# nunofachada/cl_ops

Measured on AMD Instinct MI355X. Metric: Mkeys/s sorting 2^28 uint32 (satradix, 4-bit digits); achieved % of HBM roofline, higher is better.
Workload: dtype u32

## Files before the change

cl_ops_amd/csrc/hip/clo_hip_radix1.hip:

```cpp
#include <hip/hip_runtime.h>

#include <cstdio>
#include <cstdlib>

#include "clo_hip.h"
#include "clo_hip_internal.h"
#include "clo_hip_radix_rank.h"

namespace {

constexpr int R1_PEEL = 4;
constexpr int R1_WINDOW = 8;
constexpr unsigned R1_VALID = 0x80000000u;
constexpr int R1_CNT_SHIFT = 40;
constexpr clo_u64 R1_SUM_MASK = (1ull << R1_CNT_SHIFT) - 1ull;
constexpr int R1_ROW = 256;
constexpr int R1_POOLS = 8;
constexpr int R1_TICKET_STRIDE = 16;
constexpr int R1_GH_THREADS = 512;

__device__ __forceinline__ unsigned r1_ld32(const unsigned* p) {
	return __hip_atomic_load(p, __ATOMIC_RELAXED, __HIP_MEMORY_SCOPE_AGENT);
}
__device__ __forceinline__ void r1_st32(unsigned* p, unsigned v) {
	__hip_atomic_store(p, v, __ATOMIC_RELAXED, __HIP_MEMORY_SCOPE_AGENT);
}

template <typename E, int NP>
__global__ __launch_bounds__(R1_GH_THREADS)
void clo_radix1_ghist_kernel(const E* __restrict__ in, size_t n, unsigned key_shift, unsigned key_bits,
	unsigned* __restrict__ ghist, unsigned* __restrict__ gbase, unsigned* __restrict__ done,
	int aligned, clo_keyx kx, unsigned tiles_per_group) {
	constexpr int ITEMS = sweep_shape<E>::ITEMS;
	constexpr int TILE = R1_GH_THREADS * ITEMS;
	constexpr int COPIES = NP <= 4 ? 32 : 16;
	__shared__ unsigned s_cnt[NP * (R1_ROW / 2) * COPIES];
	const unsigned tid = threadIdx.x, cp = tid & (COPIES - 1);
	for (unsigned i = tid; i < (unsigned) (NP * (R1_ROW / 2) * COPIES); i += R1_GH_THREADS) s_cnt[i] = 0;
	__syncthreads();
	const unsigned last_bits = key_bits - 8u * (NP - 1);
	const unsigned last_mask = (1u << last_bits) - 1u;
	const size_t tile0 = (size_t) blockIdx.x * tiles_per_group;
	for (unsigned t = 0; t < tiles_per_group; ++t) {
		const size_t base = (tile0 + t) * TILE;
		if (base >= n) break;
		const unsigned count = (n - base) < (size_t) TILE ? (unsigned) (n - base) : (unsigned) TILE;
		const unsigned tbase = tid * ITEMS;
		E key[ITEMS];
		if (count == (unsigned) TILE) {
			load_blocked<E, ITEMS>(in + base + tbase, key, aligned != 0);
		} else {
			#pragma unroll
			for (int i = 0; i < ITEMS; ++i) key[i] = (tbase + i < count) ? in[base + tbase + i] : (E) 0;
		}
		#pragma unroll
		for (int i = 0; i < ITEMS; ++i) {
			if (count == (unsigned) TILE || tbase + i < count) {
				const E k = clo_keyx_fwd<E>(key[i], kx) >> key_shift;
				#pragma unroll
				for (int p = 0; p < NP; ++p) {
					const unsigned d = (unsigned) (k >> (8 * p)) & (p == NP - 1 ? last_mask : 255u);
					atomicAdd(&s_cnt[((unsigned) p * (R1_ROW / 2) + (d >> 1)) * COPIES + cp], 1u << ((d & 1u) * 16u));
				}
			}
		}
	}
	__syncthreads();
	for (unsigned i = tid; i < (unsigned) (NP * R1_ROW / 2); i += R1_GH_THREADS) {
		unsigned even = 0, odd = 0;
		#pragma unroll
		for (int c = 0; c < COPIES; ++c) {
			const unsigned x = s_cnt[i * COPIES + ((c + i) & (COPIES - 1))];
			even += x & 0xffffu;
			odd += x >> 16;
		}
		if (even) atomicAdd(&ghist[2 * i], even);
		if (odd) atomicAdd(&ghist[2 * i + 1], odd);
	}
	__shared__ unsigned s_last, s_w[4];
	asm volatile("s_waitcnt vmcnt(0)" ::: "memory");
	__syncthreads();
	if (tid == 0) s_last = atomicAdd(done, 1u) == gridDim.x - 1u;
	__syncthreads();
	if (!s_last) return;
	const unsigned lane = tid & 63u, wave = tid >> 6;
	for (int p = 0; p < NP; ++p) {
		unsigned v = 0, incl = 0;
		if (tid < (unsigned) R1_ROW) {
			v = __hip_atomic_load(&ghist[p * R1_ROW + tid], __ATOMIC_RELAXED, __HIP_MEMORY_SCOPE_AGENT);
			incl = clo_wave_scan_inclusive<unsigned>(v, lane);
			if (lane == 63) s_w[wave] = incl;
		}
		__syncthreads();
		if (tid < (unsigned) R1_ROW) {
			unsigned b = incl - v;
			#pragma unroll
			for (unsigned w = 0; w < 4; ++w) if (w < wave) b += s_w[w];
			gbase[p * R1_ROW + tid] = b;
		}
		__syncthreads();
	}
}

struct r1_pass {
	unsigned* agg;
	clo_u64* cacc;
	unsigned* cprefix;
	unsigned* ticket;
	const unsigned* gbase;
	unsigned* status;
	clo_u64* stamps;
	unsigned tiles, max_spins;
	unsigned pools;
};

template <typename E, int LB, int HB, int R1_CHUNK_LOG, int R1_EARLY>
__global__ __launch_bounds__(sweep_shape<E>::THREADS, 6)
void clo_radix1_sweep_kernel(const E* __restrict__ in, E* __restrict__ out, size_t n,
	unsigned shift, unsigned mask_lo, unsigned mask_hi, r1_pass P, int aligned, clo_keyx kx_in, clo_keyx kx_out) {

	constexpr int THREADS = sweep_shape<E>::THREADS;
	constexpr int ITEMS = sweep_shape<E>::ITEMS;
	constexpr int TILE = THREADS * ITEMS;
	constexpr int WAVES = THREADS / 64;
	constexpr int R2 = 1 << (LB + HB);
	constexpr int HMAX = pc_words<(LB > HB ? LB : HB)>::H;
	constexpr unsigned R1_CHUNK = 1u << R1_CHUNK_LOG;
	static_assert(R1_EARLY <= (int) R1_CHUNK, "at most the whole level 1");
	static_assert(R2 <= R1_ROW && R2 <= THREADS, "one thread per combined digit");
	static_assert(THREADS >= 2 * R1_ROW, "the digit threads are the second half of the work-group");

	__shared__ __attribute__((aligned(16))) E s_stage[TILE];
	__shared__ unsigned s_end[THREADS * PC_END_STRIDE];
	__shared__ unsigned s_wtot[WAVES][HMAX];
	__shared__ __attribute__((aligned(16))) unsigned s_wbase[WAVES][HMAX];
	__shared__ unsigned s_delta[R2];
	__shared__ unsigned s_w4[4];
	__shared__ unsigned s_tile;

	const unsigned tid = threadIdx.x, lane = tid & 63u, wave = tid >> 6;
	clo_u64 t0 = 0, t1 = 0, t2 = 0, t3 = 0, t4 = 0, t5 = 0;
	if (P.stamps) t0 = __builtin_amdgcn_s_memtime();

	const int dg = (int) tid - (THREADS - R1_ROW);
	const bool dthread = dg >= 0 && dg < R2;
	const bool dwaves = wave >= (unsigned) (WAVES - R1_ROW / 64);
	const unsigned dwave = wave - (unsigned) (WAVES - R1_ROW / 64);

	unsigned* s_hist = reinterpret_cast<unsigned*>(s_stage);
	static_assert(sizeof(E) * TILE >= WAVES * R1_ROW * sizeof(unsigned), "the histogram fits the stage");
	#pragma unroll
	for (int k = 0; k < WAVES * R1_ROW / THREADS; ++k) s_hist[k * THREADS + tid] = 0;

	if (tid == 0) {
		const unsigned nchunks = (P.tiles + R1_CHUNK - 1u) >> R1_CHUNK_LOG;
		const unsigned x = clo_xcc_id();
		unsigned tile = 0xffffffffu;
		for (unsigned t = 0; t < P.pools; ++t) {
			const unsigned pool = (x + t) & (P.pools - 1u);
			const unsigned k = atomicAdd(&P.ticket[pool * R1_TICKET_STRIDE], 1u);
			const unsigned c = (k >> R1_CHUNK_LOG) * P.pools + pool;
			const unsigned cand = (c << R1_CHUNK_LOG) + (k & (R1_CHUNK - 1u));
			if (c < nchunks && cand < P.tiles) { tile = cand; break; }
		}
		s_tile = tile;
	}
	clo_lds_barrier();
	const unsigned tile = s_tile;
	if (tile == 0xffffffffu) return;
	const unsigned c = tile >> R1_CHUNK_LOG, q = tile & (R1_CHUNK - 1u);
	const unsigned in_chunk = P.tiles - (c << R1_CHUNK_LOG) < R1_CHUNK ? P.tiles - (c << R1_CHUNK_LOG) : R1_CHUNK;
	const size_t base = (size_t) tile * TILE;
	const unsigned count = (n - base) < (size_t) TILE ? (unsigned) (n - base) : (unsigned) TILE;
	const bool full = count == (unsigned) TILE;
	const unsigned tbase = tid * ITEMS;
	const unsigned mask2 = (mask_hi << LB) | mask_lo;
	const unsigned n32 = (unsigned) n;

	E key[ITEMS];
	if (full) {
		load_blocked<E, ITEMS>(in + base + tbase, key, aligned != 0);
	} else {
		#pragma unroll
		for (int i = 0; i < ITEMS; ++i) key[i] = (tbase + i < count) ? in[base + tbase + i] : (E) 0;
	}
	if (kx_in.kind) {
		#pragma unroll
		for (int i = 0; i < ITEMS; ++i) key[i] = clo_keyx_fwd<E>(key[i], kx_in);
	}
	if (P.stamps) t1 = __builtin_amdgcn_s_memtime();
	{
		const unsigned d0 = (unsigned) (key[0] >> shift) & mask2;
		const bool skewed = __popcll(__ballot(d0 == (unsigned) __builtin_amdgcn_readfirstlane((int) d0))) >= 16;
		unsigned* const row = s_hist + wave * R1_ROW;
		if (!skewed) {
			#pragma unroll
			for (int i = 0; i < ITEMS; ++i)
				if (full || tbase + i < count) atomicAdd(&row[(unsigned) (key[i] >> shift) & mask2], 1u);
		} else {
			#pragma unroll
			for (int i = 0; i < ITEMS; ++i) {
				const unsigned d = (unsigned) (key[i] >> shift) & mask2;
				bool mine = full || tbase + i < count;
				#pragma unroll 1
				for (int r = 0; r < R1_PEEL; ++r) {
					const unsigned long long rem = __ballot(mine);
					if (rem == 0) break;
					const int l = __ffsll((long long) rem) - 1;
					const unsigned dl = (unsigned) __builtin_amdgcn_readlane((int) d, l);
					const bool grp = mine && d == dl;
					const unsigned cnt = (unsigned) __popcll(__ballot(grp));
					if ((int) lane == l) atomicAdd(&row[dl], cnt);
					mine = mine && !grp;
				}
				if (mine) atomicAdd(&row[d], 1u);
			}
		}
	}

	unsigned h2 = 0, incl2 = 0;
	clo_u64 old = 0;
	auto publish = [&]() {
		if (!dwaves) return;
		if (dthread) {
			#pragma unroll
			for (int w = 0; w < WAVES; ++w) h2 += s_hist[w * R1_ROW + dg];
			r1_st32(&P.agg[(size_t) tile * R1_ROW + dg], R1_VALID | h2);
			old = __hip_atomic_fetch_add(&P.cacc[(size_t) c * R1_ROW + dg], (1ull << R1_CNT_SHIFT) | (clo_u64) h2,
				__ATOMIC_RELAXED, __HIP_MEMORY_SCOPE_AGENT);
		}
		incl2 = clo_wave_scan_inclusive<unsigned>(h2, lane);
		if (lane == 63) s_w4[dwave] = incl2;
	};
	pc_local_split<E, LB, THREADS, ITEMS, HMAX>(key, shift, mask_lo, count, s_stage, s_end, s_wtot, s_wbase, publish);
	if (P.stamps) t2 = __builtin_amdgcn_s_memtime();

	unsigned dstart2 = 0;
	unsigned early[R1_EARLY > 0 ? R1_EARLY : 1];
	#pragma unroll
	for (unsigned k = 0; k < (unsigned) R1_EARLY; ++k) early[k] = (k == 0 ? c > 0 : k <= q) ? 0u : R1_VALID;
	if (dthread) {
		dstart2 = incl2 - h2;
		#pragma unroll
		for (unsigned w = 0; w < 4; ++w) if (w < dwave) dstart2 += s_w4[w];
		if ((unsigned) (old >> R1_CNT_SHIFT) == in_chunk - 1u) {
			const clo_u64 total = (old & R1_SUM_MASK) + h2;
			clo_u64 excl = 0;
			long j = (long) c - 1;
			unsigned spins = 0;
			while (j >= 0) {
				unsigned pv[R1_WINDOW];
				clo_u64 av[R1_WINDOW];
				#pragma unroll
				for (int w = 0; w < R1_WINDOW; ++w) {
					pv[w] = 0; av[w] = 0;
					if (j - w >= 0) {
						pv[w] = r1_ld32(&P.cprefix[(size_t) (j - w) * R1_ROW + dg]);
						av[w] = clo_ld_agent(&P.cacc[(size_t) (j - w) * R1_ROW + dg]);
					}
				}
				bool closed = false, stalled = false;
				int used = 0;
				#pragma unroll
				for (int w = 0; w < R1_WINDOW; ++w) {
					if (closed || stalled || j - w < 0) continue;
					if (pv[w] & R1_VALID) { excl += pv[w] & ~R1_VALID; closed = true; }
					else if ((unsigned) (av[w] >> R1_CNT_SHIFT) == R1_CHUNK) { excl += av[w] & R1_SUM_MASK; used = w + 1; }
					else stalled = true;
				}
				if (closed) break;
				j -= used;
				if (stalled) {
					if (++spins > P.max_spins) { atomicExch(P.status, 1u); break; }
					__builtin_amdgcn_s_sleep(2);
				}
			}
			r1_st32(&P.cprefix[(size_t) c * R1_ROW + dg], R1_VALID | (unsigned) (excl + total));
		}
	}
	if (P.stamps) t3 = __builtin_amdgcn_s_memtime();

	if (mask_hi != 0) {
		if (full) {
			constexpr int PER = ITEMS * (int) sizeof(E) >= 16 ? 16 / (int) sizeof(E) : ITEMS;
			typedef E vec16 __attribute__((ext_vector_type(PER)));
			#pragma unroll
			for (int k = 0; k < ITEMS / PER; ++k) {
				const vec16 t = *reinterpret_cast<const vec16*>(&s_stage[tbase + k * PER]);
				#pragma unroll
				for (int qq = 0; qq < PER; ++qq) key[k * PER + qq] = t[qq];
			}
		} else {
			#pragma unroll
			for (int i = 0; i < ITEMS; ++i) if (tbase + i < count) key[i] = s_stage[tbase + i];
		}
		auto request = [&]() {
			if (!dthread) return;
			#pragma unroll
			for (unsigned k = 0; k < (unsigned) R1_EARLY; ++k) {
				const bool want = k == 0 ? c > 0 : k <= q;
				const unsigned* a = !want ? &P.agg[(size_t) tile * R1_ROW + dg]
					: (k == 0 ? &P.cprefix[(size_t) (c - 1) * R1_ROW + dg] : &P.agg[(size_t) (tile - k) * R1_ROW + dg]);
				early[k] = r1_ld32(a);
			}
		};
		pc_local_split<E, HB, THREADS, ITEMS, HMAX>(key, shift + LB, mask_hi, count, s_stage, s_end, s_wtot, s_wbase, request);
	}
	if (P.stamps) t4 = __builtin_amdgcn_s_memtime();

	if (dthread) {
		const unsigned* addr[R1_CHUNK];
		unsigned v[R1_CHUNK];
		#pragma unroll
		for (unsigned k = 0; k < R1_CHUNK; ++k) {
			const bool want = k == 0 ? c > 0 : k <= q;
			addr[k] = !want ? &P.agg[(size_t) tile * R1_ROW + dg]
				: (k == 0 ? &P.cprefix[(size_t) (c - 1) * R1_ROW + dg] : &P.agg[(size_t) (tile - k) * R1_ROW + dg]);
			v[k] = k < (unsigned) R1_EARLY ? early[k] : (want ? 0u : R1_VALID);
		}
		unsigned spins = 0;
		for (;;) {
			bool all = true;
			#pragma unroll
			for (unsigned k = 0; k < R1_CHUNK; ++k) all = all && (v[k] & R1_VALID);
			if (all) break;
			if (spins != 0) __builtin_amdgcn_s_sleep(1);
			if (++spins > P.max_spins) { atomicExch(P.status, 1u); break; }
			#pragma unroll
			for (unsigned g = 0; g < R1_CHUNK / 4; ++g) {
				if (g != 0 && q < 4 * g) continue;
				if (spins == 1 && 4 * g + 3 < (unsigned) R1_EARLY) {
					const bool have = (v[4 * g] & v[4 * g + 1] & v[4 * g + 2] & v[4 * g + 3] & R1_VALID) != 0;
					if (__builtin_amdgcn_ballot_w64(!have) == 0) continue;
				}
				unsigned nv[4];
				#pragma unroll
				for (unsigned k = 0; k < 4; ++k) nv[k] = r1_ld32(addr[4 * g + k]);
				#pragma unroll
				for (unsigned k = 0; k < 4; ++k) if (!(v[4 * g + k] & R1_VALID)) v[4 * g + k] = nv[k];
			}
		}
		#pragma unroll
		for (unsigned k = 0; k < R1_CHUNK; ++k) {
			const bool want = k == 0 ? c > 0 : k <= q;
			if (!want) v[k] = R1_VALID;
		}
		unsigned excl = 0;
		#pragma unroll
		for (unsigned k = 0; k < R1_CHUNK; ++k) excl += v[k] & ~R1_VALID;
		s_delta[dg] = P.gbase[dg] + excl - dstart2;
	}
	clo_lds_barrier();
	if (P.stamps) t5 = __builtin_amdgcn_s_memtime();

	constexpr int VEC = sizeof(E) >= 8 ? 1 : 4;
	typedef E vecE __attribute__((ext_vector_type(VEC)));
	typedef E vecE_u __attribute__((ext_vector_type(VEC), aligned(sizeof(E))));
	#pragma unroll
	for (int j = 0; j < ITEMS / VEC; ++j) {
		const unsigned p = (j * THREADS + tid) * VEC;
		if (full) {
			const vecE vv = *reinterpret_cast<const vecE*>(&s_stage[p]);
			const unsigned d0 = (unsigned) (vv[0] >> shift) & mask2, dl = (unsigned) (vv[VEC - 1] >> shift) & mask2;
			const unsigned gi0 = p + s_delta[d0];
			if (d0 == dl && gi0 <= n32 - VEC) {
				vecE vo = vv;
				if (kx_out.kind) {
					#pragma unroll
					for (int k = 0; k < VEC; ++k) vo[k] = clo_keyx_inv<E>(vv[k], kx_out);
				}
				*reinterpret_cast<vecE_u*>(&out[gi0]) = vo;
			} else {
				#pragma unroll
				for (int k = 0; k < VEC; ++k) {
					const unsigned gi = p + k + s_delta[(unsigned) (vv[k] >> shift) & mask2];
					if (gi < n32) out[gi] = clo_keyx_inv<E>(vv[k], kx_out);
				}
			}
		} else {
			#pragma unroll
			for (int k = 0; k < VEC; ++k) {
				if (p + k < count) {
					const E e = s_stage[p + k];
					const unsigned gi = p + k + s_delta[(unsigned) (e >> shift) & mask2];
					if (gi < n32) out[gi] = clo_keyx_inv<E>(e, kx_out);
				}
			}
		}
	}
	if (P.stamps && tid == 0) {
		clo_u64* st = P.stamps + (size_t) tile * 8;
		st[0] = t0; st[1] = t1; st[2] = t2; st[3] = t3; st[4] = t4; st[5] = t5;
		st[6] = __builtin_amdgcn_s_memtime();
		st[7] = ((clo_u64) clo_xcc_id() << 32) | blockIdx.x;
	}
}

struct r1_layout { size_t ghist, gbase, tickets, done, pass0, per_pass, agg, cacc, cprefix, total, tiles, chunks; int passes; };

r1_layout r1_make_layout(size_t n, int elem_size, int key_bits) {
	r1_layout L;
	const size_t tile = (size_t) 512 * (elem_size == 8 ? 8 : 16);
	L.tiles = (n + tile - 1) / tile;
	if (L.tiles == 0) L.tiles = 1;
	L.chunks = (L.tiles + 7) / 8;
	L.passes = (key_bits + 7) / 8;
	size_t off = 0;
	L.ghist = off; off += (size_t) L.passes * R1_ROW * sizeof(unsigned);
	L.gbase = off; off += (size_t) L.passes * R1_ROW * sizeof(unsigned);
	L.tickets = off; off += (size_t) L.passes * R1_POOLS * R1_TICKET_STRIDE * sizeof(unsigned);
	L.done = off; off += 64;
	off = (off + 255) & ~(size_t) 255;
	L.pass0 = off;
	L.agg = 0;
	L.cacc = L.agg + L.tiles * R1_ROW * sizeof(unsigned);
	L.cprefix = L.cacc + L.chunks * R1_ROW * sizeof(clo_u64);
	L.per_pass = (L.cprefix + L.chunks * R1_ROW * sizeof(unsigned) + 255) & ~(size_t) 255;
	L.total = L.pass0 + L.per_pass * (size_t) L.passes;
	return L;
}

int r1_device_cus() {
	int dev = 0, cus = 0;
	if (hipGetDevice(&dev) != hipSuccess) return 0;
	if (hipDeviceGetAttribute(&cus, hipDeviceAttributeMultiprocessorCount, dev) != hipSuccess) return 0;
	return cus;
}

clo_u64* g_r1_stamps = nullptr;
size_t g_r1_stamps_tiles = 0;

template <typename E, int NP>
void r1_launch_ghist(const E* src, size_t n, int key_shift, int key_bits, unsigned* ghist, unsigned* gbase, unsigned* done,
	clo_keyx kx, unsigned tiles, hipStream_t s) {
	unsigned per = tiles > 4096u ? (tiles + 2047u) / 2048u : (tiles > 256u ? 2u : 1u);
	if (per > 16u) per = 16u;
	const unsigned groups = (tiles + per - 1u) / per;
	hipLaunchKernelGGL((clo_radix1_ghist_kernel<E, NP>), dim3(groups), dim3(R1_GH_THREADS), 0, s,
		src, n, (unsigned) key_shift, (unsigned) key_bits, ghist, gbase, done, (int) ((uintptr_t) src % 16 == 0), kx, per);
}

template <typename E>
int r1_sort_impl(const E* src, E* dst, E* tmp, size_t n, int key_shift, int key_bits, clo_keyx kx, void* ws, unsigned* status, hipStream_t s) {
	const r1_layout L = r1_make_layout(n, (int) sizeof(E), key_bits);
	char* w = (char*) ws;
	unsigned* ghist = (unsigned*) (w + L.ghist);
	unsigned* gbase = (unsigned*) (w + L.gbase);
	unsigned* tickets = (unsigned*) (w + L.tickets);
	const unsigned tiles = (unsigned) L.tiles;
	const int passes = L.passes;
	const clo_keyx kx_none = { 0, 0, 0 };
	const clo_hip_env_t* env = clo_hip_env();
	const unsigned max_spins = env->max_spins;

	unsigned pools = (tiles > 1024u && r1_device_cus() >= 256) ? (unsigned) R1_POOLS : 1u;
	if (env->r1_pools != 0) pools = env->r1_pools == R1_POOLS ? (unsigned) R1_POOLS : 1u;

	hipError_t e = hipMemsetAsync(ws, 0, L.total, s);
	if (e != hipSuccess) return (int) e;
	{
		clo_timing_scope timing("radix_ghist", s);
		switch (passes) {
			#define CLO_R1_GH(NP) case NP: r1_launch_ghist<E, NP>(src, n, key_shift, key_bits, ghist, gbase, (unsigned*) (w + L.done), kx, tiles, s); break
			CLO_R1_GH(1); CLO_R1_GH(2); CLO_R1_GH(3); CLO_R1_GH(4); CLO_R1_GH(5); CLO_R1_GH(6); CLO_R1_GH(7); CLO_R1_GH(8);
			#undef CLO_R1_GH
			default: return CLO_HIP_EUNSUPPORTED;
		}
	}
	const bool inplace_odd = (dst == src) && (passes % 2 == 1);
	const E* cur_in = src;
	for (int p = 0; p < passes; ++p) {
		E* cur_out;
		if (inplace_odd) cur_out = (p % 2 == 0) ? tmp : dst;
		else cur_out = ((passes - 1 - p) % 2 == 0) ? dst : tmp;
		const int rem = key_bits - p * 8;
		const int bits = rem < 8 ? rem : 8;
		const int lo_bits = bits < 4 ? bits : 4, hi_bits = bits - lo_bits;
		char* pw = w + L.pass0 + (size_t) p * L.per_pass;
		r1_pass P;
		P.agg = (unsigned*) (pw + L.agg);
		P.cacc = (clo_u64*) (pw + L.cacc);
		P.cprefix = (unsigned*) (pw + L.cprefix);
		P.ticket = tickets + (size_t) p * R1_POOLS * R1_TICKET_STRIDE;
		P.gbase = gbase + (size_t) p * R1_ROW;
		P.status = status;
		P.stamps = (g_r1_stamps && g_r1_stamps_tiles >= L.tiles && p == passes - 1) ? g_r1_stamps : nullptr;
		P.tiles = tiles;
		P.max_spins = max_spins;
		P.pools = pools;
		clo_timing_scope timing("radix_sweep", s);
		#define CLO_R1_SWEEP(CL, EARLY) hipLaunchKernelGGL((clo_radix1_sweep_kernel<E, 4, 4, CL, EARLY>), dim3(tiles), dim3(sweep_shape<E>::THREADS), 0, s, \
			cur_in, cur_out, n, (unsigned) (key_shift + p * 8), (1u << lo_bits) - 1u, (1u << hi_bits) - 1u, P, \
			(int) ((uintptr_t) cur_in % 16 == 0), p == 0 ? kx : kx_none, p + 1 == passes ? kx : kx_none)
		CLO_R1_SWEEP(4, 8);
		#undef CLO_R1_SWEEP
		cur_in = cur_out;
	}
	e = hipGetLastError();
	if (e != hipSuccess) return (int) e;
	if (inplace_odd) {
		e = hipMemcpyAsync(dst, tmp, n * sizeof(E), hipMemcpyDeviceToDevice, s);
		if (e != hipSuccess) return (int) e;
	}
	return 0;
}

}

int clo_radix1_applies(size_t n, int elem_size, int digit_bits) {
	const int mode = clo_hip_env()->radix_sweep;
	if (mode == 0) return 0;
	if ((digit_bits != 4 && digit_bits != 8) || (elem_size != 4 && elem_size != 8) || n >= 0x80000000ull) return 0;
	const size_t tiles = (n + (size_t) 512 * (elem_size == 8 ? 8 : 16) - 1) / ((size_t) 512 * (elem_size == 8 ? 8 : 16));
	if (mode == 1) return tiles > 1;
	return tiles >= 2 && tiles <= 256;
}

size_t clo_radix1_workspace_bytes(size_t n, int elem_size, int key_bits) {
	return r1_make_layout(n, elem_size, key_bits).total;
}

int clo_radix1_sort(const void* src, void* dst, void* tmp, size_t n, int elem_size, int key_shift, int key_bits,
	clo_keyx kx, void* ws, unsigned* status, hipStream_t s) {
	if (elem_size == 4) return r1_sort_impl<uint32_t>((const uint32_t*) src, (uint32_t*) dst, (uint32_t*) tmp, n, key_shift, key_bits, kx, ws, status, s);
	if (elem_size == 8) return r1_sort_impl<uint64_t>((const uint64_t*) src, (uint64_t*) dst, (uint64_t*) tmp, n, key_shift, key_bits, kx, ws, status, s);
	return CLO_HIP_EUNSUPPORTED;
}

extern "C" int clo_hip_radix_debug_stamps(void* buffer, size_t tiles) {
	g_r1_stamps = (clo_u64*) buffer;
	g_r1_stamps_tiles = buffer ? tiles : 0;
	return 0;
}
```

cl_ops_amd/csrc/hip/clo_hip_radix4.hip:

```cpp
#include <hip/hip_runtime.h>

#include <cstdlib>
#include <type_traits>

#include "clo_hip.h"
#include "clo_hip_internal.h"
#include "clo_hip_radix_rank.h"

namespace {

template <int KB> struct kv_key;
template <> struct kv_key<1> { typedef uint8_t type; };
template <> struct kv_key<2> { typedef uint16_t type; };
template <> struct kv_key<4> { typedef uint32_t type; };

template <int KB, int ITEMS>
__device__ __forceinline__ void kv_load_pairs(const clo_kv_io& kv, size_t at, unsigned valid, bool aligned, uint64_t (&pair)[ITEMS]) {
	typedef typename kv_key<KB>::type K;
	const K* kp = reinterpret_cast<const K*>(kv.keys_in) + at;
	K k[ITEMS];
	unsigned v[ITEMS];
	if (valid == (unsigned) ITEMS) {
		load_blocked<K, ITEMS>(kp, k, aligned);
		if (kv.values_in) {
			load_blocked<unsigned, ITEMS>(kv.values_in + at, v, aligned);
		} else {
			#pragma unroll
			for (int i = 0; i < ITEMS; ++i) v[i] = (unsigned) at + (unsigned) i;
		}
	} else {
		#pragma unroll
		for (int i = 0; i < ITEMS; ++i) {
			k[i] = (unsigned) i < valid ? kp[i] : (K) 0;
			v[i] = (unsigned) i < valid ? (kv.values_in ? kv.values_in[at + i] : (unsigned) at + (unsigned) i) : 0u;
		}
	}
	#pragma unroll
	for (int i = 0; i < ITEMS; ++i) pair[i] = ((uint64_t) k[i] << 32) | v[i];
}

template <int KB>
__device__ __forceinline__ void kv_store_pair(const clo_kv_io& kv, unsigned gi, uint64_t e) {
	typedef typename kv_key<KB>::type K;
	if (kv.keys_out) reinterpret_cast<K*>(kv.keys_out)[gi] = (K) (e >> 32);
	kv.values_out[gi] = (unsigned) e;
}

template <typename E, int LB, int HB, bool BIG, bool DIG = false, bool SEG = false, int KV_IN = 0, int KV_OUT = 0>
__global__ __launch_bounds__((pair_shape<E, BIG>::THREADS), (pair_shape<E, BIG>::THREADS >= 1024 ? 8 : 6))
void clo_radix4_pair_kernel(const E* __restrict__ in, E* __restrict__ out, size_t n,
	unsigned shift, unsigned mask_lo, unsigned mask_hi,
	const unsigned* __restrict__ thist, const unsigned* __restrict__ toff, const unsigned* __restrict__ dbase,
	const unsigned* __restrict__ tinfo, int aligned,
	clo_keyx kx_in, clo_keyx kx_out, unsigned char* __restrict__ dig_out = nullptr, unsigned next_shift = 0,
	const clo_seg_tile* __restrict__ tdesc = nullptr, const E* __restrict__ in2 = nullptr, clo_kv_io kv = clo_kv_io()) {
	static_assert((KV_IN == 0 && KV_OUT == 0) || (sizeof(E) == 8 && !SEG), "key-value passes: 8-byte pairs, one array");

	constexpr int THREADS = pair_shape<E, BIG>::THREADS;
	constexpr int ITEMS = pair_shape<E, BIG>::ITEMS;
	constexpr int TILE = THREADS * ITEMS;
	constexpr int WAVES = THREADS / 64;
	constexpr int R2 = 1 << (LB + HB);
	constexpr int HMAX = pc_words<(LB > HB ? LB : HB)>::H;
	static_assert(R2 <= 256 && R2 <= THREADS, "one thread per combined digit, scanned by the first four waves");

	__shared__ __attribute__((aligned(16))) E s_stage[TILE];
	constexpr bool ALIAS = pair_shape<E, BIG>::ALIAS;
	__shared__ unsigned s_end[ALIAS ? 1 : THREADS * PC_END_STRIDE];
	__shared__ unsigned s_wtot[WAVES][HMAX];
	__shared__ __attribute__((aligned(16))) unsigned s_wbase[WAVES][HMAX];
	__shared__ unsigned s_delta[R2];
	__shared__ unsigned s_w4[4];

	const unsigned tid = threadIdx.x, lane = tid & 63u, wave = tid >> 6;
	const unsigned per_xcd = SEG ? (unsigned) ((n + 7) / 8) : (unsigned) ((n + (size_t) TILE * 8 - 1) / ((size_t) TILE * 8));
	const unsigned tile = (blockIdx.x & 7u) * per_xcd + (blockIdx.x >> 3);
	size_t base = (size_t) tile * TILE;
	unsigned count, n32;
	if constexpr (SEG) {
		if (tile >= (unsigned) n) return;
		const clo_seg_tile td = tdesc[tile];
		base = (size_t) td.in_base;
		count = td.count_seg & 0xffffu;
		n32 = td.seg_n;
		out += td.out_base;
		if constexpr (DIG) dig_out += td.out_base;
		dbase += (size_t) ((td.count_seg >> 16) & 0x7fffu) * R2;
		if (td.count_seg >> 31) in = in2;
	} else {
		if (base >= n) return;
		count = (n - base) < (size_t) TILE ? (unsigned) (n - base) : (unsigned) TILE;
		n32 = n > 0xffffffffull ? 0xffffffffu : (unsigned) n;
	}
	const bool full = count == (unsigned) TILE;
	const unsigned tbase = tid * ITEMS;
	const unsigned mask2 = (mask_hi << LB) | mask_lo;

	__builtin_amdgcn_s_setprio(3);
	unsigned h2 = 0, goff = 0;
	if (tid < (unsigned) R2) {
		h2 = thist[(size_t) tile * R2 + tid];
		goff = toff[(size_t) tile * R2 + tid];
		if (dbase) goff += dbase[tid];
	}
	E key[ITEMS];
	if constexpr (KV_IN != 0) {
		kv_load_pairs<KV_IN, ITEMS>(kv, base + tbase, full ? (unsigned) ITEMS : (count > tbase ? count - tbase : 0u), aligned != 0, key);
	} else if (full) {
		if constexpr (SEG) load_blocked_unaligned<E, ITEMS>(in + base + tbase, key);
		else load_blocked<E, ITEMS>(in + base + tbase, key, aligned != 0);
	} else {
		#pragma unroll
		for (int i = 0; i < ITEMS; ++i) key[i] = (tbase + i < count) ? in[base + tbase + i] : (E) 0;
	}
	__builtin_amdgcn_s_setprio(0);
	if (kx_in.kind) {
		#pragma unroll
		for (int i = 0; i < ITEMS; ++i) key[i] = clo_keyx_fwd<E>(key[i], kx_in);
	}
	{
		const unsigned incl2 = clo_wave_scan_inclusive<unsigned>(h2, lane);
		if (lane == 63 && wave < 4) s_w4[wave] = incl2;
		if (tid < (unsigned) R2) s_delta[tid] = goff - (incl2 - h2);
	}

	const bool single = tinfo[tile] != 0u;

	if (!single) {
		pc_local_split<E, LB, THREADS, ITEMS, HMAX, pc_no_mid, pc_no_counted, ALIAS>(key, shift, mask_lo, count, s_stage, s_end, s_wtot, s_wbase);
	} else {
		if (full) {
			constexpr int PER = ITEMS * (int) sizeof(E) >= 16 ? 16 / (int) sizeof(E) : ITEMS;
			typedef E vec16 __attribute__((ext_vector_type(PER)));
			#pragma unroll
			for (int k = 0; k < ITEMS / PER; ++k) {
				vec16 t;
				#pragma unroll
				for (int q = 0; q < PER; ++q) t[q] = key[k * PER + q];
				*reinterpret_cast<vec16*>(&s_stage[tbase + k * PER]) = t;
			}
		} else {
			#pragma unroll
			for (int i = 0; i < ITEMS; ++i) if (tbase + i < count) s_stage[tbase + i] = key[i];
		}
		clo_lds_barrier();
	}

	if (tid < (unsigned) R2) {
		unsigned before = 0;
		#pragma unroll
		for (unsigned w = 0; w < 4; ++w) if (w < wave) before += s_w4[w];
		s_delta[tid] -= before;
	}
	if (single) {
		__syncthreads();
	} else if (mask_hi != 0) {
		if (full) {
			constexpr int PER = ITEMS * (int) sizeof(E) >= 16 ? 16 / (int) sizeof(E) : ITEMS;
			typedef E vec16 __attribute__((ext_vector_type(PER)));
			#pragma unroll
			for (int k = 0; k < ITEMS / PER; ++k) {
				const vec16 t = *reinterpret_cast<const vec16*>(&s_stage[tbase + k * PER]);
				#pragma unroll
				for (int q = 0; q < PER; ++q) key[k * PER + q] = t[q];
			}
		} else {
			#pragma unroll
			for (int i = 0; i < ITEMS; ++i) if (tbase + i < count) key[i] = s_stage[tbase + i];
		}
		pc_local_split<E, HB, THREADS, ITEMS, HMAX, pc_no_mid, pc_no_counted, ALIAS>(key, shift + LB, mask_hi, count, s_stage, s_end, s_wtot, s_wbase);
	} else {
		__syncthreads();
	}

	constexpr int VEC = sizeof(E) >= 8 ? 1 : 4;
	typedef E vecE __attribute__((ext_vector_type(VEC)));
	typedef E vecE_u __attribute__((ext_vector_type(VEC), aligned(sizeof(E))));
	const bool dig_bytes = DIG && VEC == 4 && (next_shift & 7u) == 0u && next_shift < 8u * (unsigned) sizeof(E);
	const unsigned dig_b = next_shift >> 3;
	const unsigned dig_sel_lo = 0x0c0c0400u + dig_b * 0x0101u, dig_sel_hi = 0x04000c0cu + dig_b * 0x01010000u;
	const unsigned nbits2 = (unsigned) __builtin_popcount(mask2);
	const auto scatter = [&](auto kx_tag) {
		constexpr bool KX = decltype(kx_tag)::value;
		#pragma unroll
		for (int j = 0; j < ITEMS / VEC; ++j) {
			const unsigned p = (j * THREADS + tid) * VEC;
			if (full) {
				const vecE v = *reinterpret_cast<const vecE*>(&s_stage[p]);
				const unsigned d0 = pc_digit<E>(v[0], shift, mask2, nbits2), dl = pc_digit<E>(v[VEC - 1], shift, mask2, nbits2);
				const unsigned gi0 = p + s_delta[d0];
				if (d0 == dl && gi0 <= n32 - VEC) {
					vecE vo = v;
					if constexpr (KX) {
						#pragma unroll
						for (int k = 0; k < VEC; ++k) vo[k] = clo_keyx_inv<E>(v[k], kx_out);
					}
					if constexpr (KV_OUT != 0) kv_store_pair<KV_OUT>(kv, gi0, vo[0]);
					else *reinterpret_cast<vecE_u*>(&out[gi0]) = vo;
					if constexpr (DIG) {
						if constexpr (VEC == 4) {
							typedef unsigned u32_u __attribute__((aligned(1)));
							unsigned dg;
							if (dig_bytes)
								dg = __builtin_amdgcn_perm((unsigned) v[1], (unsigned) v[0], dig_sel_lo) | __builtin_amdgcn_perm((unsigned) v[3], (unsigned) v[2], dig_sel_hi);
							else
								dg = ((unsigned) (v[0] >> next_shift) & 255u) | (((unsigned) (v[1] >> next_shift) & 255u) << 8)
									| (((unsigned) (v[2] >> next_shift) & 255u) << 16) | ((unsigned) (v[3] >> next_shift) << 24);
							*reinterpret_cast<u32_u*>(dig_out + gi0) = dg;
						} else {
							dig_out[gi0] = (unsigned char) (v[0] >> next_shift);
						}
					}
				} else {
					#pragma unroll
					for (int k = 0; k < VEC; ++k) {
						const unsigned gi = p + k + s_delta[pc_digit<E>(v[k], shift, mask2, nbits2)];
						if (gi < n32) {
							if constexpr (KV_OUT != 0) kv_store_pair<KV_OUT>(kv, gi, KX ? clo_keyx_inv<E>(v[k], kx_out) : v[k]);
							else out[gi] = KX ? clo_keyx_inv<E>(v[k], kx_out) : v[k];
							if constexpr (DIG) dig_out[gi] = (unsigned char) (v[k] >> next_shift);
						}
					}
				}
			} else {
				#pragma unroll
				for (int k = 0; k < VEC; ++k) {
					if (p + k < count) {
						const E e = s_stage[p + k];
						const unsigned gi = p + k + s_delta[pc_digit<E>(e, shift, mask2, nbits2)];
						if (gi < n32) {
							if constexpr (KV_OUT != 0) kv_store_pair<KV_OUT>(kv, gi, KX ? clo_keyx_inv<E>(e, kx_out) : e);
							else out[gi] = KX ? clo_keyx_inv<E>(e, kx_out) : e;
							if constexpr (DIG) dig_out[gi] = (unsigned char) (e >> next_shift);
						}
					}
				}
			}
		}
	};
	if (kx_out.kind) scatter(std::true_type()); else scatter(std::false_type());
}

constexpr int SMALL_TILE = 512 * 8;
template <typename E> struct small_big { static constexpr int THREADS = 1024, ITEMS = sizeof(E) == 8 ? 8 : 16, TILE = THREADS * ITEMS; };

template <typename E, int BITS, int THREADS, int ITEMS>
__global__ __launch_bounds__(THREADS)
void clo_radix4_small_kernel(const E* in, E* out, unsigned n, unsigned key_shift, unsigned key_bits, clo_keyx kx) {
	constexpr int H = pc_words<BITS>::H;
	constexpr int WAVES = THREADS / 64;
	__shared__ __attribute__((aligned(16))) E s_stage[THREADS * ITEMS];
	__shared__ unsigned s_end[THREADS * PC_END_STRIDE];
	__shared__ unsigned s_wtot[WAVES][H];
	__shared__ __attribute__((aligned(16))) unsigned s_wbase[WAVES][H];

	const unsigned tbase = threadIdx.x * ITEMS;
	E key[ITEMS];
	#pragma unroll
	for (int i = 0; i < ITEMS; ++i) key[i] = (tbase + i < n) ? clo_keyx_fwd<E>(in[tbase + i], kx) : (E) 0;
	for (unsigned done = 0; done < key_bits; done += BITS) {
		const unsigned bits = key_bits - done < (unsigned) BITS ? key_bits - done : (unsigned) BITS;
		pc_local_split<E, BITS, THREADS, ITEMS, H>(key, key_shift + done, (1u << bits) - 1u, n,
			s_stage, s_end, s_wtot, s_wbase);
		if constexpr (ITEMS * sizeof(E) >= 16) {
			constexpr int PER = 16 / (int) sizeof(E);
			typedef E vec16 __attribute__((ext_vector_type(PER)));
			#pragma unroll
			for (int k = 0; k < ITEMS / PER; ++k) {
				const vec16 t = *reinterpret_cast<const vec16*>(&s_stage[tbase + k * PER]);
				#pragma unroll
				for (int q = 0; q < PER; ++q) key[k * PER + q] = t[q];
			}
		} else {
			#pragma unroll
			for (int i = 0; i < ITEMS; ++i) if (tbase + i < n) key[i] = s_stage[tbase + i];
		}
	}
	#pragma unroll
	for (int i = 0; i < ITEMS; ++i) if (tbase + i < n) out[tbase + i] = clo_keyx_inv<E>(key[i], kx);
}


struct rp_layout { size_t thist, toff, partial, tinfo, dig, total, tiles; bool big; };

rp_layout rp_make_layout(size_t n, int elem_size, int pass_bits, bool digits = true) {
	rp_layout L;
	const size_t R2 = (size_t) 1 << pass_bits;
	L.big = clo_radix_big_tiles(n, elem_size);
	const size_t tile = clo_pair_tile_elems(elem_size, L.big);
	L.tiles = (n + tile - 1) / tile;
	if (L.tiles == 0) L.tiles = 1;
	const size_t per = L.tiles * R2 * sizeof(unsigned);
	L.thist = CLO_WS_HEADER_BYTES;
	L.toff = L.thist + per;
	L.partial = L.toff + per;
	L.tinfo = L.partial + ((clo_radixw_partial_rows(L.tiles) * R2 * sizeof(unsigned) + 255) & ~(size_t) 255);
	L.total = L.tinfo + ((L.tiles * sizeof(unsigned) + 255) & ~(size_t) 255);
	L.dig = 0;
	if (digits && clo_radix_digit_stream(n, elem_size)) {
		L.dig = L.total;
		L.total += (n + 255) & ~(size_t) 255;
	}
	return L;
}

template <typename Layout>
clo_radix_counters rp_counters(void* ws, const Layout& L, size_t tiles) {
	char* w = (char*) ws;
	return { (unsigned*) (w + L.thist), (unsigned*) (w + L.toff), (unsigned*) (w + L.partial), (unsigned*) (w + L.tinfo), (unsigned) tiles, L.big };
}

struct rp_digits { unsigned shift, mask_lo, mask_hi, mask, next_shift; };

template <int LB, int HB>
rp_digits rp_pass_digits(int p, int key_shift, int key_bits) {
	constexpr int PB = LB + HB;
	const int rem = key_bits - p * PB;
	const int bits = rem < PB ? rem : PB;
	const int lo_bits = bits < LB ? bits : LB, hi_bits = bits - lo_bits;
	rp_digits d;
	d.shift = (unsigned) (key_shift + p * PB);
	d.mask_lo = (1u << lo_bits) - 1u;
	d.mask_hi = (1u << hi_bits) - 1u;
	d.mask = (d.mask_hi << LB) | d.mask_lo;
	d.next_shift = d.shift + PB;
	return d;
}

template <typename E, int LB, int HB, bool SEG = false, int KB = 0>
void rp_launch_pass(const clo_radix_counters& c, const rp_digits& d, const E* in, E* out, size_t n, const unsigned* dbase, int aligned,
	clo_keyx kx_in, clo_keyx kx_out, unsigned char* dig_out, hipStream_t s, const clo_seg_tile* tdesc = nullptr, const E* in2 = nullptr,
	bool kv_in = false, bool kv_out = false, const clo_kv_io& kv = clo_kv_io()) {
	const unsigned tiles = SEG ? (unsigned) n : c.tiles;
	const auto launch = [&](auto big, auto dig, auto kvi, auto kvo) {
		constexpr bool BIG = decltype(big)::value, DIG = decltype(dig)::value;
		hipLaunchKernelGGL((clo_radix4_pair_kernel<E, LB, HB, BIG, DIG, SEG, decltype(kvi)::value, decltype(kvo)::value>),
			dim3((tiles + 7u) / 8u * 8u), dim3(pair_shape<E, BIG>::THREADS), 0, s,
			in, out, n, d.shift, d.mask_lo, d.mask_hi, c.thist, c.toff, dbase, c.tinfo, aligned, kx_in, kx_out, dig_out, d.next_shift, tdesc, in2, kv);
	};
	const auto shape = [&](auto kvi, auto kvo) {
		constexpr bool BIG_OK = sizeof(E) >= 4, DIG_OK = BIG_OK && LB == 4 && HB == 4 && decltype(kvo)::value == 0;
		if constexpr (DIG_OK) {
			if (c.big && dig_out) { launch(std::true_type(), std::true_type(), kvi, kvo); return; }
		}
		if constexpr (BIG_OK) {
			if (c.big) { launch(std::true_type(), std::false_type(), kvi, kvo); return; }
		}
		launch(std::false_type(), std::false_type(), kvi, kvo);
	};
	typedef std::integral_constant<int, 0> plain;
	typedef std::integral_constant<int, KB> key;
	if (kv_in && kv_out) shape(key(), key());
	else if (kv_in) shape(key(), plain());
	else if (kv_out) shape(plain(), key());
	else shape(plain(), plain());
}

int kv_unpack(const uint64_t* pairs, const clo_kv_io& io, size_t n, int key_size, hipStream_t s);

template <typename E, int LB, int HB, int KB = 0>
int rp_sort_impl(const E* src, E* dst, E* tmp, size_t n, int key_shift, int key_bits, clo_keyx kx, const unsigned char* first_dig,
	const clo_kv_io& kv, void* ws, hipStream_t s) {
	constexpr int PB = LB + HB;
	const int passes = (key_bits + PB - 1) / PB;
	const rp_layout L = rp_make_layout(n, (int) sizeof(E), PB);
// ... 398 lines not shown
```

cl_ops_amd/csrc/hip/clo_hip_radix_rank.h:

```cpp
#ifndef CLO_HIP_RADIX_RANK_H
#define CLO_HIP_RADIX_RANK_H

#include <hip/hip_runtime.h>

#include <cstdlib>

#include "clo_hip_internal.h"

namespace {



template <int CTRL, int ROW_MASK>
__device__ __forceinline__ unsigned dpp_add(unsigned x) {
	return x + (unsigned) __builtin_amdgcn_update_dpp(0, (int) x, CTRL, ROW_MASK, 0xF, true);
}

constexpr int PC_BATCH = 4;
constexpr int PC_END_STRIDE = 8;

template <int BITS> struct pc_words { static constexpr int H = (1 << BITS) >= 2 ? (1 << BITS) / 2 : 1; };

template <typename E, int ITEMS>
__device__ __forceinline__ void load_blocked(const E* __restrict__ p, E (&key)[ITEMS], bool aligned) {
// ... 109 lines not shown
	if constexpr (sizeof(E) <= 4) return __builtin_amdgcn_ubfe((unsigned) key, dshift, nbits);
	else return (unsigned) (key >> dshift) & dmask;
}

struct pc_no_mid { __device__ __forceinline__ void operator()() const {} };
struct pc_no_counted { __device__ __forceinline__ void operator()(unsigned long long, unsigned long long) const {} };

template <typename E, int BITS, int THREADS, int ITEMS, int HMAX, bool FULL, bool ALIAS, typename Mid, typename Counted>
__device__ __forceinline__ void pc_local_split_impl(const E (&key)[ITEMS], unsigned dshift, unsigned dmask, unsigned count,
	E* s_stage, unsigned* s_end, unsigned (*s_wtot)[HMAX], unsigned (*s_wbase)[HMAX], Mid mid, Counted counted) {
	constexpr int H = pc_words<BITS>::H;
	constexpr int WAVES = THREADS / 64;
	const unsigned tid = threadIdx.x, lane = tid & 63u, wave = tid >> 6;
	const unsigned tbase = tid * ITEMS;

	static_assert(ITEMS == 8 || ITEMS == 16, "one or two packed counters");
	unsigned long long run = 0, c2 = 0;
	unsigned rb[ITEMS / 4];
	const unsigned nbits = (unsigned) __builtin_popcount(dmask);
	#pragma unroll
	for (int k = 0; k < ITEMS / 4; ++k) rb[k] = 0;
	#pragma unroll
	for (int i = ITEMS - 1; i >= 0; --i) {
		if (ITEMS == 16 && i == 7) c2 = run;
		if (FULL || tbase + i < count) {
			const unsigned sh = pc_digit<E>(key[i], dshift, dmask, nbits) * 4u;
			pc_put_byte(rb[i >> 2], (unsigned) (run >> sh), i & 3);
			run += 1ull << sh;
		}
	}
	const unsigned long long c = run - c2;
	constexpr unsigned ES = (unsigned) sizeof(E);
	static_assert((size_t) THREADS * ITEMS * sizeof(E) <= 65536, "byte offsets of the stage fit in 16 bits");
	#pragma unroll
	for (int k = 0; k < ITEMS / 4; ++k) rb[k] = pc_rank_bytes<(int) ES>(rb[k]);
	counted(c, c2);
	unsigned w[H];
	pc2_wave_scan<BITS, (ITEMS > 8)>(c, c2, w);
	if (lane == 63) {
		#pragma unroll
		for (int j = 0; j < H; ++j) s_wtot[wave][j] = w[j];
	}
	clo_lds_barrier();
	if (wave == 0) {
		static_assert(WAVES <= 16, "one row of 16 lanes spans the waves");

		constexpr int ROUNDS = (H + 3) / 4;
		const unsigned wv = lane & 15u, q = lane >> 4;
		unsigned excl[ROUNDS], tot[ROUNDS];
		#pragma unroll
		for (int r = 0; r < ROUNDS; ++r) {
			const unsigned j = r * 4 + q;
			const unsigned x = (j < (unsigned) H && wv < (unsigned) WAVES) ? s_wtot[wv][j] : 0u;
			unsigned incl = dpp_add<0x111, 0xF>(x);
			incl = dpp_add<0x112, 0xF>(incl);
			incl = dpp_add<0x114, 0xF>(incl);
			incl = dpp_add<0x118, 0xF>(incl);
			excl[r] = incl - x;
			tot[r] = incl;
		}
		unsigned run = 0, dstart16[H];
		#pragma unroll
		for (int j = 0; j < H; ++j) {
			const unsigned t = (unsigned) __builtin_amdgcn_readlane((int) tot[j / 4], (j % 4) * 16 + 15);
			dstart16[j] = run | ((run + (t & 0xffffu)) << 16);
			run += (t & 0xffffu) + (t >> 16);
		}
		#pragma unroll
		for (int r = 0; r < ROUNDS; ++r) {
			unsigned mine = dstart16[r * 4];
			#pragma unroll
			for (int k = 1; k < 4; ++k) if (r * 4 + k < H && q == (unsigned) k) mine = dstart16[r * 4 + k];
			const unsigned j = r * 4 + q;
			if (j < (unsigned) H && wv < (unsigned) WAVES) s_wbase[wv][j] = pc_pk_scale<(int) ES>(mine + excl[r]);
		}
	}
	mid();
	clo_lds_barrier();
	typedef unsigned short __attribute__((may_alias)) pc_u16;
	pc_u16* const tab = reinterpret_cast<pc_u16*>(s_end) + ((tid & ~63u) + ((tid & 31u) << 1) + ((tid >> 5) & 1u));
	unsigned wb[H];
	if constexpr (H % 4 == 0 && HMAX % 4 == 0) {
		typedef unsigned vec4u __attribute__((ext_vector_type(4)));
		#pragma unroll
		for (int k = 0; k < H / 4; ++k) {
			const vec4u t = reinterpret_cast<const vec4u*>(s_wbase[wave])[k];
			wb[4 * k] = t[0]; wb[4 * k + 1] = t[1]; wb[4 * k + 2] = t[2]; wb[4 * k + 3] = t[3];
		}
	} else {
		#pragma unroll
		for (int j = 0; j < H; ++j) wb[j] = s_wbase[wave][j];
	}
	#pragma unroll
	for (int j = 0; j < H; ++j) {
		const unsigned e2 = pc_pk_scale_add<(int) ES>(w[j], wb[j]);
		tab[(2 * j) * THREADS] = (unsigned short) e2;
		if (2 * j + 1 < (1 << BITS)) tab[(2 * j + 1) * THREADS] = (unsigned short) (e2 >> 16);
	}
	unsigned pos[ALIAS ? ITEMS : 1];
	char* const stage_bytes = reinterpret_cast<char*>(s_stage);
	#pragma unroll
	for (int i = 0; i < ITEMS; ++i) {
		if (FULL && i > 0 && i % PC_BATCH == 0) __builtin_amdgcn_sched_barrier(0);
		if (FULL || tbase + i < count) {
			const unsigned d = pc_digit<E>(key[i], dshift, dmask, nbits);
			const unsigned end = tab[d * THREADS];
			const unsigned at = pc_sub_byte16(end, rb[i >> 2], i & 3);
			if constexpr (ALIAS) pos[i] = at;
			else *reinterpret_cast<E*>(stage_bytes + at) = key[i];
		}
	}
	if constexpr (ALIAS) {
		clo_lds_barrier();
		#pragma unroll
		for (int i = 0; i < ITEMS; ++i)
			if (FULL || tbase + i < count) *reinterpret_cast<E*>(stage_bytes + pos[i]) = key[i];
	}
	clo_lds_barrier();
}

template <typename E, int BITS, int THREADS, int ITEMS, int HMAX, typename Mid = pc_no_mid, typename Counted = pc_no_counted, bool ALIAS = false>
__device__ __forceinline__ void pc_local_split(const E (&key)[ITEMS], unsigned dshift, unsigned dmask, unsigned count,
	E* s_stage, unsigned* s_end, unsigned (*s_wtot)[HMAX], unsigned (*s_wbase)[HMAX], Mid mid = Mid(), Counted counted = Counted()) {
	static_assert(!ALIAS || (size_t) THREADS * PC_END_STRIDE * 4 <= (size_t) THREADS * ITEMS * sizeof(E), "the table fits in the stage");
	unsigned* const tab = ALIAS ? reinterpret_cast<unsigned*>(s_stage) : s_end;
	if (count == (unsigned) (THREADS * ITEMS))
		pc_local_split_impl<E, BITS, THREADS, ITEMS, HMAX, true, ALIAS>(key, dshift, dmask, count, s_stage, tab, s_wtot, s_wbase, mid, counted);
	else
		pc_local_split_impl<E, BITS, THREADS, ITEMS, HMAX, false, ALIAS>(key, dshift, dmask, count, s_stage, tab, s_wtot, s_wbase, mid, counted);
}

__device__ __forceinline__ unsigned clo_xcc_id() {
	return (unsigned) __builtin_amdgcn_s_getreg((3 << 11) | (0 << 6) | 20) & 7u;
}

template <typename E> struct sweep_shape {
	static constexpr int THREADS = 512;
	static constexpr int ITEMS = sizeof(E) == 8 ? 8 : 16;
};

template <typename E, bool BIG> struct pair_shape {
	static constexpr int THREADS = (BIG && sizeof(E) >= 4) ? 1024 : 512;
	static constexpr int ITEMS = sizeof(E) == 8 ? 8 : 16;
	static constexpr int TILE = THREADS * ITEMS;
	static constexpr bool ALIAS = BIG && sizeof(E) >= 4;
};
inline size_t clo_big_tile_bytes(int elem_size) { return (size_t) (elem_size == 8 ? 32 : 256) << 20; }
inline bool clo_radix_big_tiles(size_t n, int elem_size) { return elem_size >= 4 && n * (size_t) elem_size >= clo_big_tile_bytes(elem_size); }
inline bool clo_radix_digit_stream(size_t n, int elem_size) { return clo_radix_big_tiles(n, elem_size); }
__host__ __device__ inline size_t clo_pair_tile_elems(int elem_size, bool big) {
	return (size_t) ((big && elem_size >= 4) ? 1024 : 512) * (elem_size == 8 ? 8 : 16);
}

}

#endif
```

Baseline: 115,900.

## Compact straddling quads per wave and scatter them lane-parallel

In the radix scatter, quads of four keys that do not share a digit (or run past the end) are no longer written element by element inside the divergent lane. Each wave records their (step, lane) indices in a per-wave LDS list using ballot and mbcnt. After a wave barrier, all 64 lanes process the listed elements together. This is meant to cut divergence in the per-element fallback path, at the cost of a small LDS buffer, a ballot per step and an extra loop.

```diff
diff --git a/cl_ops_amd/csrc/hip/clo_hip_radix1.hip b/cl_ops_amd/csrc/hip/clo_hip_radix1.hip
--- a/cl_ops_amd/csrc/hip/clo_hip_radix1.hip
+++ b/cl_ops_amd/csrc/hip/clo_hip_radix1.hip
@@ -137,6 +137,7 @@
 	__shared__ unsigned s_delta[R2];
 	__shared__ unsigned s_w4[4];
 	__shared__ unsigned s_tile;
+	__shared__ unsigned char s_strad[sizeof(E) <= 4 ? WAVES * pc_quads<ITEMS>::LIST : 1];
 
 	const unsigned tid = threadIdx.x, lane = tid & 63u, wave = tid >> 6;
 	clo_u64 t0 = 0, t1 = 0, t2 = 0, t3 = 0, t4 = 0, t5 = 0;
@@ -356,34 +357,50 @@
 	constexpr int VEC = sizeof(E) >= 8 ? 1 : 4;
 	typedef E vecE __attribute__((ext_vector_type(VEC)));
 	typedef E vecE_u __attribute__((ext_vector_type(VEC), aligned(sizeof(E))));
-	#pragma unroll
-	for (int j = 0; j < ITEMS / VEC; ++j) {
-		const unsigned p = (j * THREADS + tid) * VEC;
-		if (full) {
-			const vecE vv = *reinterpret_cast<const vecE*>(&s_stage[p]);
-			const unsigned d0 = (unsigned) (vv[0] >> shift) & mask2, dl = (unsigned) (vv[VEC - 1] >> shift) & mask2;
-			const unsigned gi0 = p + s_delta[d0];
-			if (d0 == dl && gi0 <= n32 - VEC) {
-				vecE vo = vv;
+	if (VEC == 4 && full) {
+		if constexpr (VEC == 4) {
+			const auto digit = [&](E e) { return (unsigned) (e >> shift) & mask2; };
+			const auto quad = [&](unsigned gi0, const vecE& v) {
+				vecE vo = v;
 				if (kx_out.kind) {
 					#pragma unroll
-					for (int k = 0; k < VEC; ++k) vo[k] = clo_keyx_inv<E>(vv[k], kx_out);
+					for (int k = 0; k < VEC; ++k) vo[k] = clo_keyx_inv<E>(v[k], kx_out);
 				}
 				*reinterpret_cast<vecE_u*>(&out[gi0]) = vo;
+			};
+			const auto one = [&](unsigned gi, E e) { out[gi] = clo_keyx_inv<E>(e, kx_out); };
+			pc_scatter_quads<E, THREADS, ITEMS>(s_stage, s_delta, s_strad, n32, digit, quad, one);
+		}
+	} else {
+		#pragma unroll
+		for (int j = 0; j < ITEMS / VEC; ++j) {
+			const unsigned p = (j * THREADS + tid) * VEC;
+			if (full) {
+				const vecE vv = *reinterpret_cast<const vecE*>(&s_stage[p]);
+				const unsigned d0 = (unsigned) (vv[0] >> shift) & mask2, dl = (unsigned) (vv[VEC - 1] >> shift) & mask2;
+				const unsigned gi0 = p + s_delta[d0];
+				if (d0 == dl && gi0 <= n32 - VEC) {
+					vecE vo = vv;
+					if (kx_out.kind) {
+						#pragma unroll
+						for (int k = 0; k < VEC; ++k) vo[k] = clo_keyx_inv<E>(vv[k], kx_out);
+					}
+					*reinterpret_cast<vecE_u*>(&out[gi0]) = vo;
+				} else {
+					#pragma unroll
+					for (int k = 0; k < VEC; ++k) {
+						const unsigned gi = p + k + s_delta[(unsigned) (vv[k] >> shift) & mask2];
+						if (gi < n32) out[gi] = clo_keyx_inv<E>(vv[k], kx_out);
+					}
+				}
 			} else {
 				#pragma unroll
 				for (int k = 0; k < VEC; ++k) {
-					const unsigned gi = p + k + s_delta[(unsigned) (vv[k] >> shift) & mask2];
-					if (gi < n32) out[gi] = clo_keyx_inv<E>(vv[k], kx_out);
-				}
-			}
-		} else {
-			#pragma unroll
-			for (int k = 0; k < VEC; ++k) {
-				if (p + k < count) {
-					const E e = s_stage[p + k];
-					const unsigned gi = p + k + s_delta[(unsigned) (e >> shift) & mask2];
-					if (gi < n32) out[gi] = clo_keyx_inv<E>(e, kx_out);
+					if (p + k < count) {
+						const E e = s_stage[p + k];
+						const unsigned gi = p + k + s_delta[(unsigned) (e >> shift) & mask2];
+						if (gi < n32) out[gi] = clo_keyx_inv<E>(e, kx_out);
+					}
 				}
 			}
 		}
diff --git a/cl_ops_amd/csrc/hip/clo_hip_radix4.hip b/cl_ops_amd/csrc/hip/clo_hip_radix4.hip
--- a/cl_ops_amd/csrc/hip/clo_hip_radix4.hip
+++ b/cl_ops_amd/csrc/hip/clo_hip_radix4.hip
@@ -71,6 +71,7 @@
 	__shared__ __attribute__((aligned(16))) unsigned s_wbase[WAVES][HMAX];
 	__shared__ unsigned s_delta[R2];
 	__shared__ unsigned s_w4[4];
+	__shared__ unsigned char s_strad[sizeof(E) <= 4 ? WAVES * pc_quads<ITEMS>::LIST : 1];
 
 	const unsigned tid = threadIdx.x, lane = tid & 63u, wave = tid >> 6;
 	const unsigned per_xcd = SEG ? (unsigned) ((n + 7) / 8) : (unsigned) ((n + (size_t) TILE * 8 - 1) / ((size_t) TILE * 8));
@@ -182,6 +183,35 @@
 	const unsigned nbits2 = (unsigned) __builtin_popcount(mask2);
 	const auto scatter = [&](auto kx_tag) {
 		constexpr bool KX = decltype(kx_tag)::value;
+		if constexpr (VEC == 4) {
+			if (full) {
+				const auto digit = [&](E e) { return pc_digit<E>(e, shift, mask2, nbits2); };
+				const auto quad = [&](unsigned gi0, const vecE& v) {
+					vecE vo = v;
+					if constexpr (KX) {
+						#pragma unroll
+						for (int k = 0; k < VEC; ++k) vo[k] = clo_keyx_inv<E>(v[k], kx_out);
+					}
+					*reinterpret_cast<vecE_u*>(&out[gi0]) = vo;
+					if constexpr (DIG) {
+						typedef unsigned u32_u __attribute__((aligned(1)));
+						unsigned dg;
+						if (dig_bytes)
+							dg = __builtin_amdgcn_perm((unsigned) v[1], (unsigned) v[0], dig_sel_lo) | __builtin_amdgcn_perm((unsigned) v[3], (unsigned) v[2], dig_sel_hi);
+						else
+							dg = ((unsigned) (v[0] >> next_shift) & 255u) | (((unsigned) (v[1] >> next_shift) & 255u) << 8)
+								| (((unsigned) (v[2] >> next_shift) & 255u) << 16) | ((unsigned) (v[3] >> next_shift) << 24);
+						*reinterpret_cast<u32_u*>(dig_out + gi0) = dg;
+					}
+				};
+				const auto one = [&](unsigned gi, E e) {
+					out[gi] = KX ? clo_keyx_inv<E>(e, kx_out) : e;
+					if constexpr (DIG) dig_out[gi] = (unsigned char) (e >> next_shift);
+				};
+				pc_scatter_quads<E, THREADS, ITEMS>(s_stage, s_delta, s_strad, n32, digit, quad, one);
+				return;
+			}
+		}
 		#pragma unroll
 		for (int j = 0; j < ITEMS / VEC; ++j) {
 			const unsigned p = (j * THREADS + tid) * VEC;
@@ -197,20 +227,7 @@
 					}
 					if constexpr (KV_OUT != 0) kv_store_pair<KV_OUT>(kv, gi0, vo[0]);
 					else *reinterpret_cast<vecE_u*>(&out[gi0]) = vo;
-					if constexpr (DIG) {
-						if constexpr (VEC == 4) {
-							typedef unsigned u32_u __attribute__((aligned(1)));
-							unsigned dg;
-							if (dig_bytes)
-								dg = __builtin_amdgcn_perm((unsigned) v[1], (unsigned) v[0], dig_sel_lo) | __builtin_amdgcn_perm((unsigned) v[3], (unsigned) v[2], dig_sel_hi);
-							else
-								dg = ((unsigned) (v[0] >> next_shift) & 255u) | (((unsigned) (v[1] >> next_shift) & 255u) << 8)
-									| (((unsigned) (v[2] >> next_shift) & 255u) << 16) | ((unsigned) (v[3] >> next_shift) << 24);
-							*reinterpret_cast<u32_u*>(dig_out + gi0) = dg;
-						} else {
-							dig_out[gi0] = (unsigned char) (v[0] >> next_shift);
-						}
-					}
+					if constexpr (DIG) dig_out[gi0] = (unsigned char) (v[0] >> next_shift);
 				} else {
 					#pragma unroll
 					for (int k = 0; k < VEC; ++k) {
diff --git a/cl_ops_amd/csrc/hip/clo_hip_radix_rank.h b/cl_ops_amd/csrc/hip/clo_hip_radix_rank.h
--- a/cl_ops_amd/csrc/hip/clo_hip_radix_rank.h
+++ b/cl_ops_amd/csrc/hip/clo_hip_radix_rank.h
@@ -285,6 +285,45 @@
 	return (size_t) ((big && elem_size >= 4) ? 1024 : 512) * (elem_size == 8 ? 8 : 16);
 }
 
+template <int ITEMS> struct pc_quads { static constexpr int STEPS = ITEMS / 4, LIST = STEPS * 64; };
+
+template <typename E, int THREADS, int ITEMS, typename Digit, typename Quad, typename One>
+__device__ __forceinline__ void pc_scatter_quads(const E* s_stage, const unsigned* s_delta, unsigned char* s_strad, unsigned n32,
+	Digit digit, Quad quad, One one) {
+	typedef E vec4 __attribute__((ext_vector_type(4)));
+	constexpr int STEPS = pc_quads<ITEMS>::STEPS;
+	static_assert(sizeof(E) <= 4 && ITEMS % 4 == 0 && pc_quads<ITEMS>::LIST <= 256, "a quad's (step, lane) fits in a byte");
+	const unsigned tid = threadIdx.x, lane = tid & 63u, wave = tid >> 6;
+	unsigned char* const list = s_strad + wave * (unsigned) pc_quads<ITEMS>::LIST;
+	unsigned listed = 0;
+	#pragma unroll
+	for (int j = 0; j < STEPS; ++j) {
+		const unsigned p = (j * THREADS + tid) * 4;
+		const vec4 v = *reinterpret_cast<const vec4*>(&s_stage[p]);
+		const unsigned d0 = digit(v[0]);
+		const unsigned gi0 = p + s_delta[d0];
+		const bool whole = d0 == digit(v[3]) && gi0 <= n32 - 4;
+		if (whole) quad(gi0, v);
+		const clo_u64 strad = __builtin_amdgcn_ballot_w64(!whole);
+		if (!whole) list[listed + clo_mbcnt(strad)] = (unsigned char) (j * 64 + (int) lane);
+		listed += (unsigned) __builtin_popcountll(strad);
+	}
+	__builtin_amdgcn_fence(__ATOMIC_RELEASE, "wavefront");
+	__builtin_amdgcn_wave_barrier();
+	__builtin_amdgcn_fence(__ATOMIC_ACQUIRE, "wavefront");
+	const unsigned elems = listed * 4;
+	for (unsigned e0 = 0; e0 < elems; e0 += 64) {
+		const unsigned e = e0 + lane;
+		if (e < elems) {
+			const unsigned b = list[e >> 2];
+			const unsigned p = ((b >> 6) * THREADS + (wave << 6) + (b & 63u)) * 4 + (e & 3u);
+			const E x = s_stage[p];
+			const unsigned gi = p + s_delta[digit(x)];
+			if (gi < n32) one(gi, x);
+		}
+	}
+}
+
 }
 
 #endif
```

Result: no change. 118,700 (median of 6 runs) (+2.4%).
